# rubiruchi/ofdm_uhd

Measured on AMD Instinct MI355X. Metric: OFDM symbols/sec (TX+loopback RX) @ N_fft=512; packet CRC pass rate, higher is better.
Workload: dtype f32; 1 GPU; N_fft=512, occ=200, QPSK, CP=128, synthetic AWGN channel (BASELINE configs[1]); payload_bytes=1026, symbols_per_packet=22, streams=1, iq_buffers=1, parallelism=independent streams, 1 per GPU

## Files before the change

### ofdm_uhd_amd/csrc/engine_rx.inc

```

template <typename T>
static int dev_excl_scan(ofdm_handle* h, const T* d_in, uint64_t n, T* d_out, T* d_total) {
  const uint64_t nb = (n + SCAN_BLOCK - 1) / SCAN_BLOCK;
  HIPCHK(h, h->rx.partial.ensure(sizeof(T) * std::max<uint64_t>(nb, 1)));
  T* part = h->rx.partial.as<T>();
  if (n == 0) {
    if (d_total) HIPCHK(h, hipMemsetAsync(d_total, 0, sizeof(T), h->stream));
    return OFDM_OK;
  }
  hipLaunchKernelGGL(HIP_KERNEL_NAME(k_scan_partials<T>), dim3((unsigned)nb), dim3(256), 0, h->stream, d_in, n, part);
  hipLaunchKernelGGL(HIP_KERNEL_NAME(k_scan_top<T>), dim3(1), dim3(256), 0, h->stream, part, nb, d_total);
  hipLaunchKernelGGL(HIP_KERNEL_NAME(k_scan_final<T>), dim3((unsigned)nb), dim3(256), 0, h->stream, d_in, n, part, d_out);
  HIPCHK(h, hipGetLastError());
  return OFDM_OK;
}

template <int N, bool TWL, bool TAPS>
static int launch_demod_t(ofdm_handle* h, const DemodParams& q, size_t shmem) {
  constexpr int T = N / 8, FPW = demod_fpw(N);
  if (shmem > 64 * 1024)
    HIPCHK(h, hipFuncSetAttribute(reinterpret_cast<const void*>(&k_rx_demod<N, TWL, TAPS>), hipFuncAttributeMaxDynamicSharedMemorySize,
                                  (int)shmem));
  hipLaunchKernelGGL(HIP_KERNEL_NAME(k_rx_demod<N, TWL, TAPS>), dim3((q.nframes + FPW - 1) / FPW), dim3(T * FPW), shmem, h->stream, q);
  HIPCHK(h, hipGetLastError());
  return OFDM_OK;
}
template <int N, bool TWL>
static int launch_demod_v(ofdm_handle* h, const DemodParams& q, size_t shmem) {
  const bool taps = q.tap_mode != 0 || q.tap_sampler || q.tap_fft || q.tap_acq || q.tap_sink || q.tap_demapped;
  return taps ? launch_demod_t<N, TWL, true>(h, q, shmem) : launch_demod_t<N, TWL, false>(h, q, shmem);
}

template <int N>
static int launch_demod(ofdm_handle* h, const DemodParams& q0) {
  DemodParams q = q0;
  constexpr int T = N / 8, WAVES = demod_fpw(N) * ((T + WAVE - 1) / WAVE);
  const bool grid = q.grid != nullptr;
  auto bytes = [&](bool twl, bool sm) { return (size_t)demod_lds_bytes(N, twl, sm, q.occ, q.arity, q.nmap, q.nbits, q.shift, grid); };
  constexpr int CU_WAVES = 4 * demod_waves_per_simd(N);
  auto wgs = [&](size_t b) { return std::max<size_t>(1, std::min<size_t>(std::max(1, CU_WAVES / WAVES), (160 * 1024) / b)); };
  constexpr bool base_twl = !fft_onebuf(N);
  const size_t w0 = wgs(bytes(base_twl, false));
  bool twl = base_twl;
  if constexpr (fft_onebuf(N)) twl = wgs(bytes(true, false)) == w0 && bytes(true, false) <= 160 * 1024;
  q.smap_lds = (wgs(bytes(twl, true)) == w0 && bytes(twl, true) <= 160 * 1024) ? 1 : 0;
  if (const char* e = getenv("OFDM_DEMOD_LDS")) {
    const int v = atoi(e);
    if constexpr (fft_onebuf(N)) twl = (v & 1) != 0;
    q.smap_lds = (v >> 1) & 1;
  }
  const size_t shmem = bytes(twl, q.smap_lds != 0);
  if (shmem > 160 * 1024) FAIL(h, OFDM_E_INVAL, "configuration needs more than 160 KiB of LDS in k_rx_demod");
  if constexpr (fft_onebuf(N)) {
    return twl ? launch_demod_v<N, true>(h, q, shmem) : launch_demod_v<N, false>(h, q, shmem);
  } else {
    return launch_demod_v<N, true>(h, q, shmem);
  }
}

static int run_demod(ofdm_handle* h, const DemodParams& q) {
  switch (h->N) {
    case 64: return launch_demod<64>(h, q);
    case 128: return launch_demod<128>(h, q);
    case 256: return launch_demod<256>(h, q);
    case 512: return launch_demod<512>(h, q);
    case 1024: return launch_demod<1024>(h, q);
    case 2048: return launch_demod<2048>(h, q);
    default: return launch_demod<4096>(h, q);
  }
}

enum { CT_CAND = 0, CT_OVERFLOW = 1, CT_NLO = 2, CT_NHI = 3, CT_CHAIN = 4, CT_NPEAKS = 5, CT_NSYM = 6, CT_KEYTOT = 7,
       CT_DEFR = 8 , CT_RAWTOT = 13, CT_PIECES = 14, CT_STASH = 15, CT_RECS = 16, CT_COUNT = 17 };

static int sync_params(ofdm_handle* h, uint64_t nsamples, bool cap_full, SyncParams* out) {
  RxState& rx = h->rx;
  const int N = h->N, CP = h->CP, T = SYNC_TILE;
  const uint64_t ntiles = (nsamples + T - 1) / T;
  const int tiles_per_seg = 32 * ((N + CP + T - 1) / T);
  const uint64_t egrid = std::min<uint64_t>(ntiles, 256ull * 8ull), egrid_small = std::min<uint64_t>(ntiles, 256ull * 16ull);
  const uint64_t cand_cap = (cap_full ? nsamples + nsamples / 8 : nsamples / 16) + (egrid + 16) * SYNC_CHUNK_C + egrid_small * 2048ull;
  const uint64_t piece_cap = (cap_full ? nsamples / 2 + 1 : nsamples / 128) + (egrid + egrid_small + 16) * SYNC_CHUNK_P;
  HIPCHK(h, rx.y.ensure(nsamples * sizeof(c32)));
  HIPCHK(h, rx.tile_B.ensure(ntiles * sizeof(double)));
  HIPCHK(h, rx.tile_np.ensure(ntiles * sizeof(uint32_t)));
  HIPCHK(h, rx.tile_pieces.ensure(piece_cap * sizeof(SyncPiece)));
  HIPCHK(h, rx.tile_first.ensure(ntiles * sizeof(uint64_t)));
  HIPCHK(h, rx.avg_in.ensure(ntiles * sizeof(double)));
  HIPCHK(h, rx.cand_u.ensure(cand_cap * sizeof(float)));
  HIPCHK(h, rx.cand_P.ensure(cand_cap * sizeof(c32)));
// ... 1008 lines not shown
```

### ofdm_uhd_amd/csrc/fft.h

```cpp
#pragma once
#include "common.h"

__host__ __device__ constexpr int fft_lds_points(int n) { return n + n / 8; }
__host__ __device__ constexpr bool fft_onebuf(int n) { return n >= 2048; }
__host__ __device__ constexpr int fft_lds_bufs(int n) { return fft_onebuf(n) ? 1 : 2; }
__host__ __device__ constexpr int fft_lds_bytes(int n) { return fft_lds_bufs(n) * fft_lds_points(n) * (int)sizeof(c32); }

__device__ __forceinline__ int lpad(int i) { return i + (i >> 3); }

struct FftWaveSync {
  __device__ __forceinline__ void operator()() const {
    __builtin_amdgcn_fence(__ATOMIC_RELEASE, "wavefront");
    __builtin_amdgcn_wave_barrier();
    __builtin_amdgcn_fence(__ATOMIC_ACQUIRE, "wavefront");
  }
};
struct FftBlockSync {
  __device__ __forceinline__ void operator()() const { __syncthreads(); }
};

template <bool INV>
__device__ __forceinline__ c32 mul_mi(c32 a) {
  return INV ? mk(-a.im, a.re) : mk(a.im, -a.re);
}

template <bool INV>
__device__ __forceinline__ void dft8(c32 v[8]) {
  const float h = 0.70710678118654752440f;
  c32 a0 = cadd(v[0], v[4]), a4 = csub(v[0], v[4]);
  c32 a1 = cadd(v[1], v[5]), a5 = csub(v[1], v[5]);
  c32 a2 = cadd(v[2], v[6]), a6 = csub(v[2], v[6]);
  c32 a3 = cadd(v[3], v[7]), a7 = csub(v[3], v[7]);
  if (INV) {
    a5 = mk((a5.re - a5.im) * h, (a5.re + a5.im) * h);
    a7 = mk((-a7.re - a7.im) * h, (a7.re - a7.im) * h);
  } else {
    a5 = mk((a5.re + a5.im) * h, (a5.im - a5.re) * h);
    a7 = mk((a7.im - a7.re) * h, (-a7.re - a7.im) * h);
  }
  a6 = mul_mi<INV>(a6);
  c32 b0 = cadd(a0, a2), b2 = csub(a0, a2);
// ... 130 lines not shown
__host__ __device__ constexpr int fft_tw_used(int n) { return 7 * (n / 8 - 1) + 1; }
__host__ __device__ constexpr int fft_tw_lds_points(int n) { return fft_tw_used(n) + fft_tw_used(n) / 8 + 1; }
template <int N>
struct FftTwRegs {
  static constexpr int LOG = (N == 64) ? 6 : (N == 128) ? 7 : (N == 256) ? 8 : (N == 512) ? 9 : (N == 1024) ? 10 : (N == 2048) ? 11 : 12;
  static constexpr int LS0 = (LOG % 3 == 1) ? 2 : (LOG % 3 == 2) ? 4 : 8;
  static constexpr int NP = (N == 64) ? 1 : (N >= 1024) ? 3 : 2;
  c32 w[NP][7];
  __device__ __forceinline__ void load(const c32* __restrict__ tw, int t) {
    int ls = LS0;
#pragma unroll
    for (int p = 0; p < NP; p++) {
#pragma unroll
      for (int q = 1; q < 8; q++) w[p][q - 1] = tw[(t % ls) * q * (N / (ls * 8))];
      ls *= 8;
    }
  }
  template <int NN, int LS, int R, bool INV>
  __device__ __forceinline__ c32 get(int, int q) const {
    static_assert(NN == N && R == 8, "register twiddles exist for the radix-8 passes");
    constexpr int p = (LS == LS0) ? 0 : (LS == LS0 * 8) ? 1 : 2;
    c32 v = w[p][q - 1];
    if (INV) v.im = -v.im;
    return v;
  }
  template <int NN, int LS, int R>
  __device__ __forceinline__ c32 fwd(int, int q) const {
    constexpr int p = (LS == LS0) ? 0 : (LS == LS0 * 8) ? 1 : 2;
    return w[p][q - 1];
  }
};

template <int N, int R, int LS, bool INV, bool FROM_REG, bool TO_REG, bool INPLACE = false, typename SyncFn = int,
          typename TwFn = FftTwTable, bool PK = false>
__device__ __forceinline__ void fft_pass_tw(c32 e[8], int t, const c32* src, c32* dst, const TwFn& twf, SyncFn sync = 0) {
  constexpr int T = N / 8;
  constexpr int NB = 8 / R;
  static_assert(!INPLACE || (NB == 1 && !FROM_REG && !TO_REG), "in-place passes are radix-8 middle passes");
  constexpr int STRIDE = N / R;
#pragma unroll
  for (int b = 0; b < NB; b++) {
    const int j = t + b * T;
    c32 v[R];
    static_assert(FROM_REG || STRIDE % 8 == 0, "padded read offsets need STRIDE % 8 == 0");
    const int rbase = FROM_REG ? 0 : lpad(j);
#pragma unroll
    for (int q = 0; q < R; q++) {
      if (FROM_REG)
        v[q] = e[b + q * NB];
      else
        v[q] = src[rbase + q * (STRIDE + STRIDE / 8)];
    }
    const int k = (LS == 1) ? 0 : (j % LS);
    if constexpr (PK) {
      cv pv[R];
#pragma unroll
      for (int q = 0; q < R; q++) pv[q] = cv_of(v[q]);
      if constexpr (LS > 1) {
#pragma unroll
        for (int q = 1; q < R; q++) pv[q] = pk_cmul_tw<INV>(pv[q], cv_of(twf.template fwd<N, LS, R>(k, q)));
      }
      if constexpr (R == 8) {
        dft8_pk<INV>(pv);
      } else if constexpr (R == 4) {
        dft4_pk<INV>(pv[0], pv[1], pv[2], pv[3]);
      } else {
        const cv sm = pv[0] + pv[1], df = pv[0] - pv[1];
        pv[0] = sm;
        pv[1] = df;
      }
#pragma unroll
      for (int q = 0; q < R; q++) v[q] = c32_of(pv[q]);
    } else {
      if constexpr (LS > 1) {
#pragma unroll
        for (int q = 1; q < R; q++) v[q] = cmul_f(v[q], twf.template get<N, LS, R, INV>(k, q));
      }
      if constexpr (R == 8) {
        dft8<INV>(v);
      } else if constexpr (R == 4) {
        dft4<INV>(v[0], v[1], v[2], v[3]);
      } else {
        dft2(v[0], v[1]);
      }
    }
    const int obase = (j - k) * R + k;
    static_assert(LS % 8 == 0 || 8 % LS == 0, "padded write offsets");
    const int wbase = TO_REG ? 0 : lpad(obase);
    if constexpr (INPLACE) sync();
#pragma unroll
    for (int r = 0; r < R; r++) {
      if (TO_REG)
        e[b + r * NB] = v[r];
      else
        dst[wbase + r * LS + ((r * LS) >> 3)] = v[r];
    }
  }
}

template <int N, int R, int LS, bool INV, bool FROM_REG, bool TO_REG, bool INPLACE = false, typename SyncFn = int, bool PK = false>
__device__ __forceinline__ void fft_pass(c32 e[8], int t, const c32* src, c32* dst, const c32* __restrict__ tw,
                                         SyncFn sync = 0) {
  fft_pass_tw<N, R, LS, INV, FROM_REG, TO_REG, INPLACE, SyncFn, FftTwTable, PK>(e, t, src, dst, FftTwTable{tw}, sync);
}

template <int N, bool INV, typename SyncFn, bool PK, typename TwFn>
__device__ __forceinline__ void fft_run_tw(c32 e[8], int t, c32* lds, const TwFn& tw, SyncFn sync) {
  c32* A = lds;
  c32* B = lds + fft_lds_points(N);
  if constexpr (N == 64) {
    fft_pass_tw<64, 8, 1, INV, true, false, false, SyncFn, TwFn, PK>(e, t, nullptr, A, tw, sync);
    sync();
    fft_pass_tw<64, 8, 8, INV, false, true, false, SyncFn, TwFn, PK>(e, t, A, nullptr, tw, sync);
  } else if constexpr (N == 128) {
    fft_pass_tw<128, 2, 1, INV, true, false, false, SyncFn, TwFn, PK>(e, t, nullptr, A, tw, sync);
    sync();
    fft_pass_tw<128, 8, 2, INV, false, false, false, SyncFn, TwFn, PK>(e, t, A, B, tw, sync);
    sync();
    fft_pass_tw<128, 8, 16, INV, false, true, false, SyncFn, TwFn, PK>(e, t, B, nullptr, tw, sync);
  } else if constexpr (N == 256) {
    fft_pass_tw<256, 4, 1, INV, true, false, false, SyncFn, TwFn, PK>(e, t, nullptr, A, tw, sync);
    sync();
    fft_pass_tw<256, 8, 4, INV, false, false, false, SyncFn, TwFn, PK>(e, t, A, B, tw, sync);
    sync();
    fft_pass_tw<256, 8, 32, INV, false, true, false, SyncFn, TwFn, PK>(e, t, B, nullptr, tw, sync);
  } else if constexpr (N == 512) {
    fft_pass_tw<512, 8, 1, INV, true, false, false, SyncFn, TwFn, PK>(e, t, nullptr, A, tw, sync);
    sync();
// ... 5 lines not shown
    sync();
    fft_pass_tw<1024, 8, 2, INV, false, false, false, SyncFn, TwFn, PK>(e, t, A, B, tw, sync);
    sync();
    fft_pass_tw<1024, 8, 16, INV, false, false, false, SyncFn, TwFn, PK>(e, t, B, A, tw, sync);
    sync();
    fft_pass_tw<1024, 8, 128, INV, false, true, false, SyncFn, TwFn, PK>(e, t, A, nullptr, tw, sync);
  } else if constexpr (N == 2048) {
    (void)B;
    fft_pass_tw<2048, 4, 1, INV, true, false, false, SyncFn, TwFn, PK>(e, t, nullptr, A, tw, sync);
    sync();
    fft_pass_tw<2048, 8, 4, INV, false, false, true, SyncFn, TwFn, PK>(e, t, A, A, tw, sync);
    sync();
    fft_pass_tw<2048, 8, 32, INV, false, false, true, SyncFn, TwFn, PK>(e, t, A, A, tw, sync);
    sync();
    fft_pass_tw<2048, 8, 256, INV, false, true, false, SyncFn, TwFn, PK>(e, t, A, nullptr, tw, sync);
  } else {
    static_assert(N == 4096, "unsupported FFT length");
    (void)B;
    fft_pass_tw<4096, 8, 1, INV, true, false, false, SyncFn, TwFn, PK>(e, t, nullptr, A, tw, sync);
    sync();
    fft_pass_tw<4096, 8, 8, INV, false, false, true, SyncFn, TwFn, PK>(e, t, A, A, tw, sync);
    sync();
    fft_pass_tw<4096, 8, 64, INV, false, false, true, SyncFn, TwFn, PK>(e, t, A, A, tw, sync);
    sync();
    fft_pass_tw<4096, 8, 512, INV, false, true, false, SyncFn, TwFn, PK>(e, t, A, nullptr, tw, sync);
  }
}

template <int N, bool INV, typename SyncFn, bool PK = false>
__device__ __forceinline__ void fft_run(c32 e[8], int t, c32* lds, const c32* __restrict__ tw, SyncFn sync) {
  fft_run_tw<N, INV, SyncFn, PK, FftTwTable>(e, t, lds, FftTwTable{tw}, sync);
}

template <int N, bool INV, bool PK = false, typename SyncFn = int, typename TwFn = FftTwTable>
__device__ __forceinline__ void fft_run1(c32 e[8], int t, c32* A, const TwFn& tw, SyncFn sync) {
  sync();
  if constexpr (N == 64) {
    fft_pass_tw<64, 8, 1, INV, true, false, false, SyncFn, TwFn, PK>(e, t, nullptr, A, tw, sync);
    sync();
    fft_pass_tw<64, 8, 8, INV, false, true, false, SyncFn, TwFn, PK>(e, t, A, nullptr, tw, sync);
  } else if constexpr (N == 128) {
    fft_pass_tw<128, 2, 1, INV, true, false, false, SyncFn, TwFn, PK>(e, t, nullptr, A, tw, sync);
    sync();
    fft_pass_tw<128, 8, 2, INV, false, false, true, SyncFn, TwFn, PK>(e, t, A, A, tw, sync);
    sync();
    fft_pass_tw<128, 8, 16, INV, false, true, false, SyncFn, TwFn, PK>(e, t, A, nullptr, tw, sync);
  } else if constexpr (N == 256) {
    fft_pass_tw<256, 4, 1, INV, true, false, false, SyncFn, TwFn, PK>(e, t, nullptr, A, tw, sync);
    sync();
    fft_pass_tw<256, 8, 4, INV, false, false, true, SyncFn, TwFn, PK>(e, t, A, A, tw, sync);
    sync();
    fft_pass_tw<256, 8, 32, INV, false, true, false, SyncFn, TwFn, PK>(e, t, A, nullptr, tw, sync);
  } else if constexpr (N == 512) {
    fft_pass_tw<512, 8, 1, INV, true, false, false, SyncFn, TwFn, PK>(e, t, nullptr, A, tw, sync);
    sync();
    fft_pass_tw<512, 8, 8, INV, false, false, true, SyncFn, TwFn, PK>(e, t, A, A, tw, sync);
    sync();
    fft_pass_tw<512, 8, 64, INV, false, true, false, SyncFn, TwFn, PK>(e, t, A, nullptr, tw, sync);
  } else if constexpr (N == 1024) {
    fft_pass_tw<1024, 2, 1, INV, true, false, false, SyncFn, TwFn, PK>(e, t, nullptr, A, tw, sync);
    sync();
    fft_pass_tw<1024, 8, 2, INV, false, false, true, SyncFn, TwFn, PK>(e, t, A, A, tw, sync);
    sync();
    fft_pass_tw<1024, 8, 16, INV, false, false, true, SyncFn, TwFn, PK>(e, t, A, A, tw, sync);
    sync();
    fft_pass_tw<1024, 8, 128, INV, false, true, false, SyncFn, TwFn, PK>(e, t, A, nullptr, tw, sync);
  } else {
    static_assert(N <= 1024, "fft_run1 is built for the channel filter's lengths; fft_run handles N >= 2048 in one buffer");
  }
}
```

### ofdm_uhd_amd/csrc/rx_demod.h

```cpp
#pragma once
#include "common.h"
#include "fft.h"
#ifndef DEMOD_PK
#define DEMOD_PK true
#endif
#include "host_util.h"

#define RAW_SLOT 4096

enum { FR_BAD_HEADER = 0, FR_COMPLETE = 1, FR_INCOMPLETE = 2 };

struct FrameResult {
  uint32_t status;
  uint32_t packetlen;
  uint32_t end_frame;
  uint32_t header_ok;
};

struct FramesParams {
  uint64_t npeaks, nsamples;
  int N, L;
  uint32_t timeout;
  float sens;
  const uint64_t* peaks;
// ... 106 lines not shown
  const double* Phi;
  const double* step;
  const uint32_t* K;
  const uint64_t* sym_base;
  const c32* tw;
  const c32* ks;
  const float* kd;
  const int16_t* smap;
  int smap_lds;
  const c32* constellation;
  const SlicerGrid* grid;
  const uint8_t* invalid;
  FrameResult* res;
  uint8_t* raw;
  c32* tap_sampler;
  c32* tap_fft;
  c32* tap_acq;
  c32* tap_sink;
  uint8_t* tap_demapped;
  int ref_on;
  int64_t ref_peak;
  double ref_phi, ref_step;
};

__host__ __device__ inline int demod_symbits_words(int nmap, int nbits) { return (nmap * nbits + 8 + 31) / 32 + 2; }
__host__ __device__ inline int demod_hinv_len(int n, int occ, int shift) {
  const int need = (occ + 2 * shift + 2 + 1) / 2;
  return need > occ ? need : occ;
}
__host__ __device__ inline int demod_red_floats(int n) { return n / 8 == WAVE ? 0 : 64; }
#ifndef DEMOD_FPW
#define DEMOD_FPW 4
#endif
__host__ __device__ constexpr int demod_fpw(int n) { return n / 8 == WAVE ? DEMOD_FPW : 1; }
__host__ __device__ inline int demod_lds_shared(int n, bool twl, bool smap_lds, int arity, int nmap, bool grid) {
  const int b = (twl ? fft_tw_lds_points(n) : 0) * (int)sizeof(c32) + arity * (int)sizeof(c32) +
                (grid ? (int)sizeof(SlicerGrid) : 0) + (smap_lds ? ((nmap * 2 + 3) & ~3) : 0);
  return (b + 15) & ~15;
}
__host__ __device__ inline int demod_lds_frame(int n, int occ, int nmap, int nbits, int shift) {
  const int b = fft_lds_points(n) * (int)sizeof(c32) + (demod_hinv_len(n, occ, shift) + occ) * (int)sizeof(c32) +
                demod_red_floats(n) * (int)sizeof(float) + ((demod_symbits_words(nmap, nbits) + 3) & ~3) * 4;
  return (b + 15) & ~15;
}
__host__ __device__ inline int demod_lds_bytes(int n, bool twl, bool smap_lds, int occ, int arity, int nmap, int nbits, int shift,
                                               bool grid) {
  return demod_lds_shared(n, twl, smap_lds, arity, nmap, grid) + demod_fpw(n) * demod_lds_frame(n, occ, nmap, nbits, shift);
}

__device__ __forceinline__ void wave_sum2_tree(float& a, float& b) {
  float t0, t1;
  asm volatile(
      "v_mov_b32 %2, %0\n\t"
      "v_mov_b32 %3, %1\n\t"
      "s_nop 1\n\t"
      "v_permlane32_swap_b32 %0, %2\n\t"
      "v_permlane32_swap_b32 %1, %3\n\t"
      "s_nop 1\n\t"
      "v_add_f32 %0, %0, %2\n\t"
      "v_add_f32 %1, %1, %3\n\t"
      "v_mov_b32 %2, %0\n\t"
      "v_mov_b32 %3, %1\n\t"
      "s_nop 1\n\t"
      "v_permlane16_swap_b32 %0, %2\n\t"
      "v_permlane16_swap_b32 %1, %3\n\t"
      "s_nop 1\n\t"
      "v_add_f32 %0, %0, %2\n\t"
      "v_add_f32 %1, %1, %3\n\t"
      "s_nop 1\n\t"
      "v_add_f32_dpp %2, %0, %0 row_shl:8 row_mask:0xf bank_mask:0x3\n\t"
      "v_add_f32_dpp %2, %0, %0 row_shr:8 row_mask:0xf bank_mask:0xc\n\t"
      "v_add_f32_dpp %3, %1, %1 row_shl:8 row_mask:0xf bank_mask:0x3\n\t"
      "v_add_f32_dpp %3, %1, %1 row_shr:8 row_mask:0xf bank_mask:0xc\n\t"
      "s_nop 1\n\t"
      "v_add_f32_dpp %0, %2, %2 row_shl:4 row_mask:0xf bank_mask:0x5\n\t"
      "v_add_f32_dpp %0, %2, %2 row_shr:4 row_mask:0xf bank_mask:0xa\n\t"
      "v_add_f32_dpp %1, %3, %3 row_shl:4 row_mask:0xf bank_mask:0x5\n\t"
      "v_add_f32_dpp %1, %3, %3 row_shr:4 row_mask:0xf bank_mask:0xa\n\t"
      "s_nop 1\n\t"
      "v_add_f32_dpp %2, %0, %0 quad_perm:[2,3,0,1] row_mask:0xf bank_mask:0xf\n\t"
// ... 94 lines not shown
  c = fma(z, c, 4.16666666666666019037e-02);
  const double cs = fma(z * z, c, fma(-0.5, z, 1.0));
  dc o;
  o.im = (q & 1) ? cs : sn;
  o.re = (q & 1) ? -sn : cs;
  if (q & 2) {
    o.im = -o.im;
    o.re = -o.re;
  }
  return o;
}

#ifdef SYNC_STAMPS
__device__ unsigned long long g_demod_stamps[16];
#define DSTAMP(i)                                                        \
  do {                                                                   \
    if (threadIdx.x == 0) {                                              \
      __builtin_amdgcn_s_waitcnt(0xC07F);                                \
      const unsigned long long now_ = __builtin_amdgcn_s_memtime();     \
      __builtin_amdgcn_s_waitcnt(0xC07F);                                \
      dst_acc[i] += now_ - dst_last;                                     \
      dst_last = now_;                                                   \
    }                                                                    \
  } while (0)
#else
#define DSTAMP(i) do { } while (0)
#endif
#ifndef DEMOD_WAVES
#define DEMOD_WAVES 4
#endif
#ifndef DEMOD_WAVES_BIG
#define DEMOD_WAVES_BIG 4
#endif
__host__ __device__ constexpr int demod_waves_per_simd(int n) { return (n / 8 >= 256) ? DEMOD_WAVES_BIG : DEMOD_WAVES; }
template <int FPW>
__device__ __forceinline__ void frame_sync() {
  if constexpr (FPW > 1) {
    FftWaveSync()();
  } else {
    __syncthreads();
  }
}
template <int N, bool TWL, bool TAPS>
__global__ void __launch_bounds__(((N / 8 < 64) ? 64 : N / 8) * demod_fpw(N), demod_waves_per_simd(N)) k_rx_demod(DemodParams q_in) {
  DemodParams q = q_in;
  if constexpr (!TAPS) {
    q.tap_sampler = nullptr;
    q.tap_fft = nullptr;
    q.tap_acq = nullptr;
    q.tap_sink = nullptr;
    q.tap_demapped = nullptr;
    q.tap_mode = 0;
  }
  static_assert(TWL || fft_onebuf(N), "up to N = 1024 the twiddles are always in LDS");
  constexpr int T = N / 8;
  constexpr int FPW = demod_fpw(N);
  extern __shared__ __align__(16) unsigned char smem[];
  const bool use_grid = q.grid != nullptr;
  c32* twl = reinterpret_cast<c32*>(smem);
  c32* cst = twl + (TWL ? fft_tw_lds_points(N) : 0);
  SlicerGrid* grid = reinterpret_cast<SlicerGrid*>(cst + q.arity);
  int16_t* smapL = reinterpret_cast<int16_t*>(reinterpret_cast<unsigned char*>(grid) + (q.grid ? sizeof(SlicerGrid) : 0));
  const int slot = FPW > 1 ? __builtin_amdgcn_readfirstlane((int)(threadIdx.x / T)) : 0;
  unsigned char* mine = smem + demod_lds_shared(N, TWL, q.smap_lds != 0, q.arity, q.nmap, use_grid) +
                        slot * demod_lds_frame(N, q.occ, q.nmap, q.nbits, q.shift);
  c32* fftbuf = reinterpret_cast<c32*>(mine);
  c32* Ysh = fftbuf;
  c32* hinv = fftbuf + fft_lds_points(N);
  float* sd = reinterpret_cast<float*>(hinv);
  c32* dfe = hinv + demod_hinv_len(N, q.occ, q.shift);
  float* red = reinterpret_cast<float*>(dfe + q.occ);
  uint32_t* sbits = reinterpret_cast<uint32_t*>(red + demod_red_floats(N));
  const int sbw = demod_symbits_words(q.nmap, q.nbits);

  const int t = FPW > 1 ? (int)(threadIdx.x % T) : (int)threadIdx.x;
  const uint32_t f = blockIdx.x * FPW + (uint32_t)slot;
  const uint32_t q_nframes = dyn_nframes(q.dyn, q.nframes), q_j0 = dyn_j0(q.dyn, q.j0);

  {
    const int nthr = FPW * T, th = threadIdx.x;
    for (int i = th; i < q.arity; i += nthr) cst[i] = q.constellation[i];
    if constexpr (TWL)
      for (int i = th; i < fft_tw_used(N); i += nthr) twl[lpad(i)] = q.tw[i];
    if (q.smap_lds)
      for (int i = th; i < q.nmap; i += nthr) smapL[i] = q.smap[i];
    if (use_grid)
      for (int i = th; i < (int)(sizeof(SlicerGrid) / 4); i += nthr)
        reinterpret_cast<uint32_t*>(grid)[i] = reinterpret_cast<const uint32_t*>(q.grid)[i];
  }
  __syncthreads();
  if (f >= q_nframes) return;
  if (q.tap_mode && q.invalid[f]) return;

  int sstate = 0;
  float pll_phase = 0.f, pll_freq = 0.f;
  uint32_t nbits_total = 0;
  uint32_t hdr = 0, hdr_bytes = 0;
  uint32_t packetlen = 0, header_ok = 0;
  bool done = false;
  uint32_t status = FR_INCOMPLETE;
  uint32_t end_frame = f;
// ... 60 lines not shown
          Ap = dexpj(q.ref_phi + q.ref_step * (double)((int64_t)(s00 + (uint64_t)tl) - q.ref_peak + 1));
          RTp = dexpj(q.ref_step * (double)T);
        }
        dc r = Ap;
#pragma unroll
        for (int m = 0; m < 8; m++) {
          c32 rot = mk((float)r.re, (float)r.im);
          if (tl + m * T == N - 1) rot = mk((float)Rflag.re, (float)Rflag.im);
          e[m] = cmul(e[m], rot);
          r = dmul(r, RTp);
        }
      } else {
#pragma unroll
        for (int m = 0; m < 8; m++) {
          const uint64_t n = s00 + (uint64_t)(tl + m * T);
          int64_t i = (int64_t)j;
          while (i >= 0 && q.peaks[i] > n) i--;
          double ph = 0.0;
          if (i >= 0)
            ph = q.Phi[i] + q.step[i] * (double)(n - q.peaks[i] + 1);
          else if (q.ref_on)
            ph = q.ref_phi + q.ref_step * (double)((int64_t)n - q.ref_peak + 1);
          const dc r = dexpj(ph);
          e[m] = cmul(e[m], mk((float)r.re, (float)r.im));
        }
      }
      DSTAMP(1);
      if (q.tap_sampler) {
#pragma unroll
        for (int m = 0; m < 8; m++) q.tap_sampler[(symb + k) * (uint64_t)N + (uint64_t)(tl + m * T)] = e[m];
      }
      if constexpr (!fft_onebuf(N)) {
        if constexpr (FPW > 1)
          fft_run1<N, false, DEMOD_PK, FftWaveSync, FftTwLds>(e, tl, fftbuf, FftTwLds{twl}, FftWaveSync());
        else
          fft_run1<N, false, DEMOD_PK, FftBlockSync, FftTwLds>(e, tl, fftbuf, FftTwLds{twl}, FftBlockSync());
      } else if constexpr (TWL) {
        fft_run_tw<N, false, FftBlockSync, DEMOD_PK, FftTwLds>(e, tl, fftbuf, FftTwLds{twl}, FftBlockSync());
      } else {
        fft_run<N, false, FftBlockSync, DEMOD_PK>(e, tl, fftbuf, q.tw, FftBlockSync());
      }
      DSTAMP(2);
      if (k < K) {
        const uint64_t s1 = s00 + (uint64_t)(k + 1) * (uint64_t)q.L;
#pragma unroll
        for (int m = 0; m < 8; m++) nx[m] = q.y[s1 + (uint64_t)(tl + m * T)];
      }
      frame_sync<FPW>();
#pragma unroll
      for (int m = 0; m < 8; m++) Ysh[(tl + m * T + N / 2) & (N - 1)] = e[m];
      frame_sync<FPW>();
      if (q.tap_fft) {
#pragma unroll
        for (int m = 0; m < 8; m++) q.tap_fft[(symb + k) * (uint64_t)N + (uint64_t)(tl + m * T)] = Ysh[tl + m * T];
      }

      DSTAMP(3);
      if (k == 0) {
        phase_count = 1;
        const int sbase = q.zl - q.shift, slen = q.occ + 2 * q.shift;
        for (int r = t; r < slen; r += T) {
          const int i = sbase + r;
          float v = 0.f;
          if (i >= 0 && i < N - 2) v = cnorm(csub(Ysh[i], Ysh[i + 2]));
          sd[r] = v;
        }
        frame_sync<FPW>();
        int index = 0;
        float mx = 0.f;
// ... 45 lines not shown
          const float af = (float)a;
          float sn, cs;
          det_sincosf(af, &sn, &cs);
          comp = mk(f32_uniform(cs), f32_uniform(sn));
        } else {
          comp = mk(1.0f, 0.0f);
        }
        phase_count++;
        if (phase_count == 1000) phase_count = 1;
      }
      if (q.tap_acq) {
        for (int i = t; i < q.occ; i += T) {
          const int yi = i + q.zl + coarse;
          const c32 Y = (yi >= 0 && yi < N) ? Ysh[yi] : mk(0.f, 0.f);
          q.tap_acq[(symb + k) * (uint64_t)q.occ + (uint64_t)i] = cmul(cmul(hinv[i], comp), Y);
        }
      }

      DSTAMP(4);
      if (done) {
        frame_sync<FPW>();
        continue;
      }
      if (sstate == 0) {
        sstate = 1;
        frame_sync<FPW>();
        continue;
      }
      c32 carrier;
      det_sincosf(pll_phase, &carrier.im, &carrier.re);
      carrier = mk(f32_uniform(carrier.re), f32_uniform(carrier.im));
      float are = 0.f, aim = 0.f;
      const uint32_t carry_bits = nbits_total & 7u;
      for (int c = t; c < q.nmap; c += T) {
        int i;
        if (q.smap_lds)
          i = ((const __attribute__((address_space(3))) int16_t*)smapL)[c];
        else
          i = ((const __attribute__((address_space(1))) int16_t*)q.smap)[c];
        const int yi = i + q.zl + coarse;
        const c32 Y = (yi >= 0 && yi < N) ? Ysh[yi] : mk(0.f, 0.f);
        const c32 in = cmul(cmul(hinv[i], comp), Y);
        const c32 sigrot = cmul(cmul(in, carrier), dfe[c]);
        unsigned best = 0;
        float bestd;
        const float sre = fabsf(sigrot.re), sim = fabsf(sigrot.im);
        if (q.sign_kind != 0 && sre > q.sign_eps && sre < q.sign_bound && sim < q.sign_bound &&
            (q.sign_kind == 1 || sim > q.sign_eps)) {
          const bool rp = sigrot.re > 0.0f, ip = sigrot.im > 0.0f;
          if (q.sign_kind == 1)
            best = rp ? sidx1 : sidx0;
          else
            best = rp ? (ip ? sidx3 : sidx2) : (ip ? sidx1 : sidx0);
        } else if (use_grid && sre <= grid->bound && sim <= grid->bound) {
          int ka = 0, kb = 0;
          for (int a = 1; a < grid->nr - 1; a++) ka += (sigrot.re >= grid->lr[a]) ? 1 : 0;
          for (int b = 1; b < grid->ni - 1; b++) kb += (sigrot.im >= grid->li[b]) ? 1 : 0;
          best = grid->idx[ka * grid->ni + kb];
          bestd = cnorm(csub(sigrot, cst[best]));
#pragma unroll
          for (int c4 = 1; c4 < 4; c4++) {
            const unsigned cand = grid->idx[(ka + (c4 >> 1)) * grid->ni + kb + (c4 & 1)];
            const float dd = cnorm(csub(sigrot, cst[cand]));
            if (dd < bestd || (dd == bestd && cand < best)) {
              bestd = dd;
              best = cand;
            }
          }
        } else {
          bestd = cnorm(csub(sigrot, cst[0]));
          for (int jj = 1; jj < q.arity; jj++) {
            const float dd = cnorm(csub(sigrot, cst[jj]));
            if (dd < bestd) {
              bestd = dd;
              best = (unsigned)jj;
            }
          }
        }
        const c32 closest = cst[best];
        const c32 er = cmul_conj(sigrot, closest);
        are = are + er.re;
        aim = aim + er.im;
        const float sden = cnorm(sigrot);
        if (sden > 0.001f) {
          const float sinv = 1.0f / sden;
          const c32 qq = mk((closest.re * sigrot.re + closest.im * sigrot.im) * sinv,
                            (closest.im * sigrot.re - closest.re * sigrot.im) * sinv);
          c32 d = dfe[c];
          d.re = d.re + q.eq_gain * (qq.re - d.re);
          d.im = d.im + q.eq_gain * (qq.im - d.im);
          dfe[c] = d;
        }
        if (q.tap_sink) q.tap_sink[(symb + k) * (uint64_t)q.occ + (uint64_t)c] = sigrot;
        const uint32_t bp = carry_bits + (uint32_t)c * (uint32_t)q.nbits;
        atomicOr(&sbits[bp >> 5], best << (bp & 31));
        if ((bp & 31) + (uint32_t)q.nbits > 32u) atomicOr(&sbits[(bp >> 5) + 1], best >> (32 - (bp & 31)));
      }
      DSTAMP(5);
      if (q.tap_demapped && t == 0) q.tap_demapped[symb + k] = 1;
      block_sum2_f<T>(are, aim, red);
      const float angle = det_atan2f(aim, are);
      pll_freq = pll_freq - q.freq_gain * angle;
      pll_phase = pll_phase + pll_freq - q.phase_gain * angle;
      if (pll_phase >= 6.28318530717958647692f) pll_phase -= 6.28318530717958647692f;
      if (pll_phase < 0.0f) pll_phase += 6.28318530717958647692f;
      pll_phase = f32_uniform(pll_phase);
      pll_freq = f32_uniform(pll_freq);
      frame_sync<FPW>();
      const uint32_t byte0 = nbits_total >> 3;
      nbits_total += (uint32_t)q.nmap * (uint32_t)q.nbits;
      const uint32_t nbytes = nbits_total >> 3;
      const uint32_t nnew = nbytes - byte0;
      const uint8_t* sb8 = reinterpret_cast<const uint8_t*>(sbits);
      for (uint32_t b = byte0; b < nbytes && b < 4; b++) {
        hdr = (uint32_t)__builtin_amdgcn_readfirstlane((int)((hdr << 8) | sb8[b - byte0]));
        hdr_bytes++;
      }
      if (sstate == 1 && hdr_bytes == 4) {
        if (((hdr >> 16) ^ (hdr & 0xFFFF)) == 0) {
          header_ok = 1;
          packetlen = (hdr >> 16) & 0x0FFF;
          sstate = 2;
        } else {
          status = FR_BAD_HEADER;
          done = true;
          end_frame = cf;
        }
      }
      if (sstate == 2) {
// ... 296 lines not shown
```

Before: 134.9 million OFDM symbols/s.

## Add lean demod variant with wider LDS padding, packed cmul, DPP bit packing

Adds a lean configuration of the RX demod kernel used when no taps are enabled at N=512, with its own frames-per-workgroup and waves-per-SIMD settings. In that mode the FFT LDS padding stride goes from 1-in-8 to 1-in-16. It also replaces the complex multiplies in the demap loop with packed v_pk_mul/v_pk_add inline assembly, and builds each output bit word with DPP row shifts instead of one LDS atomicOr per subcarrier. The aims are fewer LDS atomics, fewer ALU instructions and less LDS bank conflict, at the cost of harder-to-read inline asm, more template variants, and possible bank conflicts from the sparser padding.

```diff
diff --git a/ofdm_uhd_amd/csrc/engine_rx.inc b/ofdm_uhd_amd/csrc/engine_rx.inc
--- a/ofdm_uhd_amd/csrc/engine_rx.inc
+++ b/ofdm_uhd_amd/csrc/engine_rx.inc
@@ -17,7 +17,7 @@
 
 template <int N, bool TWL, bool TAPS>
 static int launch_demod_t(ofdm_handle* h, const DemodParams& q, size_t shmem) {
-  constexpr int T = N / 8, FPW = demod_fpw(N);
+  constexpr int T = N / 8, FPW = demod_fpw(N, TAPS);
   if (shmem > 64 * 1024)
     HIPCHK(h, hipFuncSetAttribute(reinterpret_cast<const void*>(&k_rx_demod<N, TWL, TAPS>), hipFuncAttributeMaxDynamicSharedMemorySize,
                                   (int)shmem));
@@ -25,19 +25,16 @@
   HIPCHK(h, hipGetLastError());
   return OFDM_OK;
 }
-template <int N, bool TWL>
-static int launch_demod_v(ofdm_handle* h, const DemodParams& q, size_t shmem) {
-  const bool taps = q.tap_mode != 0 || q.tap_sampler || q.tap_fft || q.tap_acq || q.tap_sink || q.tap_demapped;
-  return taps ? launch_demod_t<N, TWL, true>(h, q, shmem) : launch_demod_t<N, TWL, false>(h, q, shmem);
-}
-
-template <int N>
-static int launch_demod(ofdm_handle* h, const DemodParams& q0) {
+
+template <int N, bool TAPS>
+static int launch_demod_l(ofdm_handle* h, const DemodParams& q0) {
   DemodParams q = q0;
-  constexpr int T = N / 8, WAVES = demod_fpw(N) * ((T + WAVE - 1) / WAVE);
+  constexpr int T = N / 8, WAVES = demod_fpw(N, TAPS) * ((T + WAVE - 1) / WAVE);
   const bool grid = q.grid != nullptr;
-  auto bytes = [&](bool twl, bool sm) { return (size_t)demod_lds_bytes(N, twl, sm, q.occ, q.arity, q.nmap, q.nbits, q.shift, grid); };
-  constexpr int CU_WAVES = 4 * demod_waves_per_simd(N);
+  auto bytes = [&](bool twl, bool sm) {
+    return (size_t)demod_lds_bytes(N, TAPS, twl, sm, q.occ, q.arity, q.nmap, q.nbits, q.shift, grid);
+  };
+  constexpr int CU_WAVES = 4 * demod_waves_per_simd(N, TAPS);
   auto wgs = [&](size_t b) { return std::max<size_t>(1, std::min<size_t>(std::max(1, CU_WAVES / WAVES), (160 * 1024) / b)); };
   constexpr bool base_twl = !fft_onebuf(N);
   const size_t w0 = wgs(bytes(base_twl, false));
@@ -52,10 +49,15 @@
   const size_t shmem = bytes(twl, q.smap_lds != 0);
   if (shmem > 160 * 1024) FAIL(h, OFDM_E_INVAL, "configuration needs more than 160 KiB of LDS in k_rx_demod");
   if constexpr (fft_onebuf(N)) {
-    return twl ? launch_demod_v<N, true>(h, q, shmem) : launch_demod_v<N, false>(h, q, shmem);
+    return twl ? launch_demod_t<N, true, TAPS>(h, q, shmem) : launch_demod_t<N, false, TAPS>(h, q, shmem);
   } else {
-    return launch_demod_v<N, true>(h, q, shmem);
-  }
+    return launch_demod_t<N, true, TAPS>(h, q, shmem);
+  }
+}
+template <int N>
+static int launch_demod(ofdm_handle* h, const DemodParams& q) {
+  const bool taps = q.tap_mode != 0 || q.tap_sampler || q.tap_fft || q.tap_acq || q.tap_sink || q.tap_demapped;
+  return taps ? launch_demod_l<N, true>(h, q) : launch_demod_l<N, false>(h, q);
 }
 
 static int run_demod(ofdm_handle* h, const DemodParams& q) {
diff --git a/ofdm_uhd_amd/csrc/fft.h b/ofdm_uhd_amd/csrc/fft.h
--- a/ofdm_uhd_amd/csrc/fft.h
+++ b/ofdm_uhd_amd/csrc/fft.h
@@ -1,12 +1,14 @@
 #pragma once
 #include "common.h"
 
-__host__ __device__ constexpr int fft_lds_points(int n) { return n + n / 8; }
+__host__ __device__ constexpr int fft_lds_points(int n, int pl = 3) { return n + (n >> pl); }
 __host__ __device__ constexpr bool fft_onebuf(int n) { return n >= 2048; }
 __host__ __device__ constexpr int fft_lds_bufs(int n) { return fft_onebuf(n) ? 1 : 2; }
 __host__ __device__ constexpr int fft_lds_bytes(int n) { return fft_lds_bufs(n) * fft_lds_points(n) * (int)sizeof(c32); }
 
 __device__ __forceinline__ int lpad(int i) { return i + (i >> 3); }
+template <int PL>
+__device__ __forceinline__ int lpad_n(int i) { return i + (i >> PL); }
 
 struct FftWaveSync {
   __device__ __forceinline__ void operator()() const {
@@ -203,7 +205,7 @@
 };
 
 template <int N, int R, int LS, bool INV, bool FROM_REG, bool TO_REG, bool INPLACE = false, typename SyncFn = int,
-          typename TwFn = FftTwTable, bool PK = false>
+          typename TwFn = FftTwTable, bool PK = false, int PL = 3>
 __device__ __forceinline__ void fft_pass_tw(c32 e[8], int t, const c32* src, c32* dst, const TwFn& twf, SyncFn sync = 0) {
   constexpr int T = N / 8;
   constexpr int NB = 8 / R;
@@ -213,14 +215,15 @@
   for (int b = 0; b < NB; b++) {
     const int j = t + b * T;
     c32 v[R];
-    static_assert(FROM_REG || STRIDE % 8 == 0, "padded read offsets need STRIDE % 8 == 0");
-    const int rbase = FROM_REG ? 0 : lpad(j);
+    constexpr int P = 1 << PL;
+    static_assert(FROM_REG || STRIDE % P == 0, "padded read offsets need STRIDE % P == 0");
+    const int rbase = FROM_REG ? 0 : lpad_n<PL>(j);
 #pragma unroll
     for (int q = 0; q < R; q++) {
       if (FROM_REG)
         v[q] = e[b + q * NB];
       else
-        v[q] = src[rbase + q * (STRIDE + STRIDE / 8)];
+        v[q] = src[rbase + q * (STRIDE + STRIDE / P)];
     }
     const int k = (LS == 1) ? 0 : (j % LS);
     if constexpr (PK) {
@@ -256,15 +259,15 @@
       }
     }
     const int obase = (j - k) * R + k;
-    static_assert(LS % 8 == 0 || 8 % LS == 0, "padded write offsets");
-    const int wbase = TO_REG ? 0 : lpad(obase);
+    static_assert(LS % P == 0 || (P % LS == 0 && ((LS * R) % P == 0 || P % (LS * R) == 0)), "padded write offsets");
+    const int wbase = TO_REG ? 0 : lpad_n<PL>(obase);
     if constexpr (INPLACE) sync();
 #pragma unroll
     for (int r = 0; r < R; r++) {
       if (TO_REG)
         e[b + r * NB] = v[r];
       else
-        dst[wbase + r * LS + ((r * LS) >> 3)] = v[r];
+        dst[wbase + r * LS + ((r * LS) >> PL)] = v[r];
     }
   }
 }
@@ -336,39 +339,39 @@
   fft_run_tw<N, INV, SyncFn, PK, FftTwTable>(e, t, lds, FftTwTable{tw}, sync);
 }
 
-template <int N, bool INV, bool PK = false, typename SyncFn = int, typename TwFn = FftTwTable>
+template <int N, bool INV, bool PK = false, typename SyncFn = int, typename TwFn = FftTwTable, int PL = 3>
 __device__ __forceinline__ void fft_run1(c32 e[8], int t, c32* A, const TwFn& tw, SyncFn sync) {
   sync();
   if constexpr (N == 64) {
-    fft_pass_tw<64, 8, 1, INV, true, false, false, SyncFn, TwFn, PK>(e, t, nullptr, A, tw, sync);
-    sync();
-    fft_pass_tw<64, 8, 8, INV, false, true, false, SyncFn, TwFn, PK>(e, t, A, nullptr, tw, sync);
+    fft_pass_tw<64, 8, 1, INV, true, false, false, SyncFn, TwFn, PK, PL>(e, t, nullptr, A, tw, sync);
+    sync();
+    fft_pass_tw<64, 8, 8, INV, false, true, false, SyncFn, TwFn, PK, PL>(e, t, A, nullptr, tw, sync);
   } else if constexpr (N == 128) {
-    fft_pass_tw<128, 2, 1, INV, true, false, false, SyncFn, TwFn, PK>(e, t, nullptr, A, tw, sync);
-    sync();
-    fft_pass_tw<128, 8, 2, INV, false, false, true, SyncFn, TwFn, PK>(e, t, A, A, tw, sync);
-    sync();
-    fft_pass_tw<128, 8, 16, INV, false, true, false, SyncFn, TwFn, PK>(e, t, A, nullptr, tw, sync);
+    fft_pass_tw<128, 2, 1, INV, true, false, false, SyncFn, TwFn, PK, PL>(e, t, nullptr, A, tw, sync);
+    sync();
+    fft_pass_tw<128, 8, 2, INV, false, false, true, SyncFn, TwFn, PK, PL>(e, t, A, A, tw, sync);
+    sync();
+    fft_pass_tw<128, 8, 16, INV, false, true, false, SyncFn, TwFn, PK, PL>(e, t, A, nullptr, tw, sync);
   } else if constexpr (N == 256) {
-    fft_pass_tw<256, 4, 1, INV, true, false, false, SyncFn, TwFn, PK>(e, t, nullptr, A, tw, sync);
-    sync();
-    fft_pass_tw<256, 8, 4, INV, false, false, true, SyncFn, TwFn, PK>(e, t, A, A, tw, sync);
-    sync();
-    fft_pass_tw<256, 8, 32, INV, false, true, false, SyncFn, TwFn, PK>(e, t, A, nullptr, tw, sync);
+    fft_pass_tw<256, 4, 1, INV, true, false, false, SyncFn, TwFn, PK, PL>(e, t, nullptr, A, tw, sync);
+    sync();
+    fft_pass_tw<256, 8, 4, INV, false, false, true, SyncFn, TwFn, PK, PL>(e, t, A, A, tw, sync);
+    sync();
+    fft_pass_tw<256, 8, 32, INV, false, true, false, SyncFn, TwFn, PK, PL>(e, t, A, nullptr, tw, sync);
   } else if constexpr (N == 512) {
-    fft_pass_tw<512, 8, 1, INV, true, false, false, SyncFn, TwFn, PK>(e, t, nullptr, A, tw, sync);
-    sync();
-    fft_pass_tw<512, 8, 8, INV, false, false, true, SyncFn, TwFn, PK>(e, t, A, A, tw, sync);
-    sync();
-    fft_pass_tw<512, 8, 64, INV, false, true, false, SyncFn, TwFn, PK>(e, t, A, nullptr, tw, sync);
+    fft_pass_tw<512, 8, 1, INV, true, false, false, SyncFn, TwFn, PK, PL>(e, t, nullptr, A, tw, sync);
+    sync();
+    fft_pass_tw<512, 8, 8, INV, false, false, true, SyncFn, TwFn, PK, PL>(e, t, A, A, tw, sync);
+    sync();
+    fft_pass_tw<512, 8, 64, INV, false, true, false, SyncFn, TwFn, PK, PL>(e, t, A, nullptr, tw, sync);
   } else if constexpr (N == 1024) {
-    fft_pass_tw<1024, 2, 1, INV, true, false, false, SyncFn, TwFn, PK>(e, t, nullptr, A, tw, sync);
-    sync();
-    fft_pass_tw<1024, 8, 2, INV, false, false, true, SyncFn, TwFn, PK>(e, t, A, A, tw, sync);
-    sync();
-    fft_pass_tw<1024, 8, 16, INV, false, false, true, SyncFn, TwFn, PK>(e, t, A, A, tw, sync);
-    sync();
-    fft_pass_tw<1024, 8, 128, INV, false, true, false, SyncFn, TwFn, PK>(e, t, A, nullptr, tw, sync);
+    fft_pass_tw<1024, 2, 1, INV, true, false, false, SyncFn, TwFn, PK, PL>(e, t, nullptr, A, tw, sync);
+    sync();
+    fft_pass_tw<1024, 8, 2, INV, false, false, true, SyncFn, TwFn, PK, PL>(e, t, A, A, tw, sync);
+    sync();
+    fft_pass_tw<1024, 8, 16, INV, false, false, true, SyncFn, TwFn, PK, PL>(e, t, A, A, tw, sync);
+    sync();
+    fft_pass_tw<1024, 8, 128, INV, false, true, false, SyncFn, TwFn, PK, PL>(e, t, A, nullptr, tw, sync);
   } else {
     static_assert(N <= 1024, "fft_run1 is built for the channel filter's lengths; fft_run handles N >= 2048 in one buffer");
   }
diff --git a/ofdm_uhd_amd/csrc/rx_demod.h b/ofdm_uhd_amd/csrc/rx_demod.h
--- a/ofdm_uhd_amd/csrc/rx_demod.h
+++ b/ofdm_uhd_amd/csrc/rx_demod.h
@@ -162,20 +162,28 @@
 #ifndef DEMOD_FPW
 #define DEMOD_FPW 4
 #endif
-__host__ __device__ constexpr int demod_fpw(int n) { return n / 8 == WAVE ? DEMOD_FPW : 1; }
+#ifndef DEMOD_FPW_LEAN
+#define DEMOD_FPW_LEAN 4
+#endif
+__host__ __device__ constexpr bool demod_lean(int n, bool taps) { return n / 8 == WAVE && !taps; }
+__host__ __device__ constexpr int demod_fpw(int n, bool taps) {
+  return n / 8 == WAVE ? (demod_lean(n, taps) ? DEMOD_FPW_LEAN : DEMOD_FPW) : 1;
+}
+__host__ __device__ constexpr int demod_pad_log(int n, bool taps) { return demod_lean(n, taps) ? 4 : 3; }
 __host__ __device__ inline int demod_lds_shared(int n, bool twl, bool smap_lds, int arity, int nmap, bool grid) {
   const int b = (twl ? fft_tw_lds_points(n) : 0) * (int)sizeof(c32) + arity * (int)sizeof(c32) +
                 (grid ? (int)sizeof(SlicerGrid) : 0) + (smap_lds ? ((nmap * 2 + 3) & ~3) : 0);
   return (b + 15) & ~15;
 }
-__host__ __device__ inline int demod_lds_frame(int n, int occ, int nmap, int nbits, int shift) {
-  const int b = fft_lds_points(n) * (int)sizeof(c32) + (demod_hinv_len(n, occ, shift) + occ) * (int)sizeof(c32) +
+__host__ __device__ inline int demod_lds_frame(int n, bool taps, int occ, int nmap, int nbits, int shift) {
+  const int b = fft_lds_points(n, demod_pad_log(n, taps)) * (int)sizeof(c32) + (demod_hinv_len(n, occ, shift) + occ) * (int)sizeof(c32) +
                 demod_red_floats(n) * (int)sizeof(float) + ((demod_symbits_words(nmap, nbits) + 3) & ~3) * 4;
   return (b + 15) & ~15;
 }
-__host__ __device__ inline int demod_lds_bytes(int n, bool twl, bool smap_lds, int occ, int arity, int nmap, int nbits, int shift,
-                                               bool grid) {
-  return demod_lds_shared(n, twl, smap_lds, arity, nmap, grid) + demod_fpw(n) * demod_lds_frame(n, occ, nmap, nbits, shift);
+__host__ __device__ inline int demod_lds_bytes(int n, bool taps, bool twl, bool smap_lds, int occ, int arity, int nmap, int nbits,
+                                               int shift, bool grid) {
+  return demod_lds_shared(n, twl, smap_lds, arity, nmap, grid) +
+         demod_fpw(n, taps) * demod_lds_frame(n, taps, occ, nmap, nbits, shift);
 }
 
 __device__ __forceinline__ void wave_sum2_tree(float& a, float& b) {
@@ -336,7 +344,33 @@
 #ifndef DEMOD_WAVES_BIG
 #define DEMOD_WAVES_BIG 4
 #endif
-__host__ __device__ constexpr int demod_waves_per_simd(int n) { return (n / 8 >= 256) ? DEMOD_WAVES_BIG : DEMOD_WAVES; }
+#ifndef DEMOD_WAVES_LEAN
+#define DEMOD_WAVES_LEAN 4
+#endif
+__host__ __device__ constexpr int demod_waves_per_simd(int n, bool taps) {
+  return (n / 8 >= 256) ? DEMOD_WAVES_BIG : demod_lean(n, taps) ? DEMOD_WAVES_LEAN : DEMOD_WAVES;
+}
+__device__ __forceinline__ c32 pk_cmul(c32 a, c32 b) {
+  cv t, u, r;
+  asm("v_pk_mul_f32 %0, %1, %2 op_sel_hi:[0,1]" : "=v"(t) : "v"(cv_of(a)), "v"(cv_of(b)));
+  asm("v_pk_mul_f32 %0, %1, %2 op_sel:[1,1] op_sel_hi:[1,0]" : "=v"(u) : "v"(cv_of(a)), "v"(cv_of(b)));
+  asm("v_pk_add_f32 %0, %1, %2 neg_lo:[0,1]" : "=v"(r) : "v"(t), "v"(u));
+  return c32_of(r);
+}
+__device__ __forceinline__ c32 pk_cmul_u(c32 a, c32 b) {
+  cv t, u, r;
+  asm("v_pk_mul_f32 %0, %1, %2 op_sel_hi:[0,1]" : "=v"(t) : "v"(cv_of(a)), "s"(cv_of(b)));
+  asm("v_pk_mul_f32 %0, %1, %2 op_sel:[1,1] op_sel_hi:[1,0]" : "=v"(u) : "v"(cv_of(a)), "s"(cv_of(b)));
+  asm("v_pk_add_f32 %0, %1, %2 neg_lo:[0,1]" : "=v"(r) : "v"(t), "v"(u));
+  return c32_of(r);
+}
+__device__ __forceinline__ c32 pk_cmul_conj(c32 a, c32 b) {
+  cv t, u, r;
+  asm("v_pk_mul_f32 %0, %1, %2 op_sel_hi:[1,0]" : "=v"(t) : "v"(cv_of(a)), "v"(cv_of(b)));
+  asm("v_pk_mul_f32 %0, %1, %2 op_sel:[1,1] op_sel_hi:[0,1]" : "=v"(u) : "v"(cv_of(a)), "v"(cv_of(b)));
+  asm("v_pk_add_f32 %0, %1, %2 neg_hi:[0,1]" : "=v"(r) : "v"(t), "v"(u));
+  return c32_of(r);
+}
 template <int FPW>
 __device__ __forceinline__ void frame_sync() {
   if constexpr (FPW > 1) {
@@ -346,7 +380,8 @@
   }
 }
 template <int N, bool TWL, bool TAPS>
-__global__ void __launch_bounds__(((N / 8 < 64) ? 64 : N / 8) * demod_fpw(N), demod_waves_per_simd(N)) k_rx_demod(DemodParams q_in) {
+__global__ void __launch_bounds__(((N / 8 < 64) ? 64 : N / 8) * demod_fpw(N, TAPS), demod_waves_per_simd(N, TAPS))
+    k_rx_demod(DemodParams q_in) {
   DemodParams q = q_in;
   if constexpr (!TAPS) {
     q.tap_sampler = nullptr;
@@ -358,7 +393,8 @@
   }
   static_assert(TWL || fft_onebuf(N), "up to N = 1024 the twiddles are always in LDS");
   constexpr int T = N / 8;
-  constexpr int FPW = demod_fpw(N);
+  constexpr int FPW = demod_fpw(N, TAPS);
+  constexpr int PL = demod_pad_log(N, TAPS);
   extern __shared__ __align__(16) unsigned char smem[];
   const bool use_grid = q.grid != nullptr;
   c32* twl = reinterpret_cast<c32*>(smem);
@@ -367,10 +403,10 @@
   int16_t* smapL = reinterpret_cast<int16_t*>(reinterpret_cast<unsigned char*>(grid) + (q.grid ? sizeof(SlicerGrid) : 0));
   const int slot = FPW > 1 ? __builtin_amdgcn_readfirstlane((int)(threadIdx.x / T)) : 0;
   unsigned char* mine = smem + demod_lds_shared(N, TWL, q.smap_lds != 0, q.arity, q.nmap, use_grid) +
-                        slot * demod_lds_frame(N, q.occ, q.nmap, q.nbits, q.shift);
+                        slot * demod_lds_frame(N, TAPS, q.occ, q.nmap, q.nbits, q.shift);
   c32* fftbuf = reinterpret_cast<c32*>(mine);
   c32* Ysh = fftbuf;
-  c32* hinv = fftbuf + fft_lds_points(N);
+  c32* hinv = fftbuf + fft_lds_points(N, PL);
   float* sd = reinterpret_cast<float*>(hinv);
   c32* dfe = hinv + demod_hinv_len(N, q.occ, q.shift);
   float* red = reinterpret_cast<float*>(dfe + q.occ);
@@ -497,9 +533,9 @@
       }
       if constexpr (!fft_onebuf(N)) {
         if constexpr (FPW > 1)
-          fft_run1<N, false, DEMOD_PK, FftWaveSync, FftTwLds>(e, tl, fftbuf, FftTwLds{twl}, FftWaveSync());
+          fft_run1<N, false, DEMOD_PK, FftWaveSync, FftTwLds, PL>(e, tl, fftbuf, FftTwLds{twl}, FftWaveSync());
         else
-          fft_run1<N, false, DEMOD_PK, FftBlockSync, FftTwLds>(e, tl, fftbuf, FftTwLds{twl}, FftBlockSync());
+          fft_run1<N, false, DEMOD_PK, FftBlockSync, FftTwLds, PL>(e, tl, fftbuf, FftTwLds{twl}, FftBlockSync());
       } else if constexpr (TWL) {
         fft_run_tw<N, false, FftBlockSync, DEMOD_PK, FftTwLds>(e, tl, fftbuf, FftTwLds{twl}, FftBlockSync());
       } else {
@@ -611,6 +647,10 @@
       carrier = mk(f32_uniform(carrier.re), f32_uniform(carrier.im));
       float are = 0.f, aim = 0.f;
       const uint32_t carry_bits = nbits_total & 7u;
+#ifndef DEMOD_WORDPACK
+#define DEMOD_WORDPACK 1
+#endif
+      const int wnb = (DEMOD_WORDPACK && T % WAVE == 0 && (q.nbits == 1 || q.nbits == 2)) ? q.nbits : 0;
       for (int c = t; c < q.nmap; c += T) {
         int i;
         if (q.smap_lds)
@@ -619,8 +659,8 @@
           i = ((const __attribute__((address_space(1))) int16_t*)q.smap)[c];
         const int yi = i + q.zl + coarse;
         const c32 Y = (yi >= 0 && yi < N) ? Ysh[yi] : mk(0.f, 0.f);
-        const c32 in = cmul(cmul(hinv[i], comp), Y);
-        const c32 sigrot = cmul(cmul(in, carrier), dfe[c]);
+        const c32 in = pk_cmul(pk_cmul_u(hinv[i], comp), Y);
+        const c32 sigrot = pk_cmul(pk_cmul_u(in, carrier), dfe[c]);
         unsigned best = 0;
         float bestd;
         const float sre = fabsf(sigrot.re), sim = fabsf(sigrot.im);
@@ -637,7 +677,7 @@
           for (int b = 1; b < grid->ni - 1; b++) kb += (sigrot.im >= grid->li[b]) ? 1 : 0;
           best = grid->idx[ka * grid->ni + kb];
           bestd = cnorm(csub(sigrot, cst[best]));
-#pragma unroll
+  #pragma unroll
           for (int c4 = 1; c4 < 4; c4++) {
             const unsigned cand = grid->idx[(ka + (c4 >> 1)) * grid->ni + kb + (c4 & 1)];
             const float dd = cnorm(csub(sigrot, cst[cand]));
@@ -657,7 +697,7 @@
           }
         }
         const c32 closest = cst[best];
-        const c32 er = cmul_conj(sigrot, closest);
+        const c32 er = pk_cmul_conj(sigrot, closest);
         are = are + er.re;
         aim = aim + er.im;
         const float sden = cnorm(sigrot);
@@ -671,9 +711,23 @@
           dfe[c] = d;
         }
         if (q.tap_sink) q.tap_sink[(symb + k) * (uint64_t)q.occ + (uint64_t)c] = sigrot;
-        const uint32_t bp = carry_bits + (uint32_t)c * (uint32_t)q.nbits;
-        atomicOr(&sbits[bp >> 5], best << (bp & 31));
-        if ((bp & 31) + (uint32_t)q.nbits > 32u) atomicOr(&sbits[(bp >> 5) + 1], best >> (32 - (bp & 31)));
+        if (wnb && __builtin_amdgcn_readfirstlane(c) + (WAVE - 1) < q.nmap) {
+          const int lane = t & (WAVE - 1);
+          uint32_t wv = best << ((lane * wnb) & 31);
+          wv |= (uint32_t)__builtin_amdgcn_update_dpp(0, (int)wv, 0x111, 0xf, 0xf, false);
+          wv |= (uint32_t)__builtin_amdgcn_update_dpp(0, (int)wv, 0x112, 0xf, 0xf, false);
+          wv |= (uint32_t)__builtin_amdgcn_update_dpp(0, (int)wv, 0x114, 0xf, 0xf, false);
+          wv |= (uint32_t)__builtin_amdgcn_update_dpp(0, (int)wv, 0x118, 0xf, 0xf, false);
+          if ((lane & 15) == 15 && wv != 0) {
+            const uint32_t w = ((uint32_t)c * (uint32_t)wnb) >> 5;
+            atomicOr(&sbits[w], wv << carry_bits);
+            if (carry_bits && (wv >> (32 - carry_bits)) != 0) atomicOr(&sbits[w + 1], wv >> (32 - carry_bits));
+          }
+        } else {
+          const uint32_t bp = carry_bits + (uint32_t)c * (uint32_t)q.nbits;
+          atomicOr(&sbits[bp >> 5], best << (bp & 31));
+          if ((bp & 31) + (uint32_t)q.nbits > 32u) atomicOr(&sbits[(bp >> 5) + 1], best >> (32 - (bp & 31)));
+        }
       }
       DSTAMP(5);
       if (q.tap_demapped && t == 0) q.tap_demapped[symb + k] = 1;
```

After: 134.1 million OFDM symbols/s (median of 3 runs). No clear change (-0.5%).
